# ratt-ru/pfb-clean

Hardware: AMD Instinct MI355X
Metric: PCG matvecs/sec (FFT-conv A^H A apply), 4k x 4k x 8-band cube (higher is better)
Workload: dtype f32; 1 GPU; 4096x4096x8-band cube PCG (hessian_psf + Tikhonov, M = x/sigmainv, tol=0, minit=maxit=20); nx_psf=8192, bands_per_gpu=8, parallelism=band-shard x1, allreduce_hook=False

## Files before the change

### include/pfb_hip.h

```cpp
#ifndef PFB_HIP_H
#define PFB_HIP_H

#include <stddef.h>
#include <stdint.h>

#ifdef __cplusplus
extern "C" {
#endif

#define PFB_ABI_VERSION 1

#define PFB_F32 0
#define PFB_F64 1

#define PFB_OK               0
#define PFB_ERR_INVALID     -1
#define PFB_ERR_UNSUPPORTED -2
#define PFB_ERR_HIP         -3
#define PFB_ERR_NONFINITE   -4
#define PFB_ERR_ALLOC       -5
#define PFB_ERR_COMM        -6

#define PFB_PCG_CONVERGED     0
#define PFB_PCG_MAXIT         1
// ... 60 lines not shown
    double rnorm;
} pfb_pcg_result;

size_t pfb_pcg_work_bytes(const pfb_conv_plan* plan, int nb);
int pfb_pcg_solve(pfb_conv_plan* plan, int band0, int nb,
                  const void* b, void* x, void* r_out,
                  const void* beam, double wsum, double sigmainv, double mdiv,
                  double tol, int maxit, int minit, int backtrack,
                  void* work, pfb_allreduce_fn allreduce, void* allreduce_ctx,
                  pfb_pcg_result* result, void* stream);

size_t pfb_pcg_bands_work_bytes(const pfb_conv_plan* plan, int nb);
int pfb_pcg_solve_bands(pfb_conv_plan* plan, int band0, int nb,
                        const void* b, void* x, void* r_out,
                        const void* beam, double wsum, double sigmainv, double mdiv,
                        double tol, int maxit, int minit, int backtrack,
                        void* work, pfb_pcg_result* results, void* stream);

int pfb_bandmix_dots(int dtype, const void* A, const void* c, int nband, size_t npix, double sigmainv,
                     const void* p, const void* r, void* out, double* dots3, double* ws, void* stream);

size_t pfb_hessparam_work_bytes(const pfb_conv_plan* plan);
int pfb_hessparam_apply(pfb_conv_plan* plan, const void* L, const void* LH, const void* e, double sigmainv,
                        const void* x, void* out, void* work, void* stream);
int pfb_hessparam_apply_dots(pfb_conv_plan* plan, const void* L, const void* LH, const void* e, double sigmainv,
                             const void* x, void* out, const void* dot_with, const void* dot_with2,
                             double* dots_out, void* work, void* stream);

size_t pfb_pcg_param_work_bytes(const pfb_conv_plan* plan, int nb);
int pfb_pcg_solve_param(pfb_conv_plan* plan, int nb, const void* L, const void* LH, const void* e,
                        const void* b, void* x, void* r_out, double sigmainv, double mdiv,
                        double tol, int maxit, int minit, int backtrack,
                        void* work, pfb_pcg_result* result, void* stream);

#define PFB_COMM_ID_BYTES 128
typedef struct pfb_comm pfb_comm;
int pfb_comm_bind(const char* librccl_path);
int pfb_comm_unique_id(void* id128);
int pfb_comm_init(int rank, int nranks, const void* id128, pfb_comm** out);
int pfb_comm_destroy(pfb_comm* comm);
int pfb_comm_info(const pfb_comm* comm, int* rank, int* nranks, int* device, int* rccl_version);
int pfb_comm_allreduce(void* comm, double* dev_buf, int count, void* stream);
int pfb_comm_check(pfb_comm* comm);
int pfb_comm_abort(pfb_comm* comm);

typedef struct pfb_psi_plan pfb_psi_plan;

int pfb_psi_plan_create(int nband, int nx, int ny, int nbasis, const int* basis_k,
                        const double* filters, int nlevel, int dtype,
                        pfb_psi_plan** plan);
int pfb_psi_plan_destroy(pfb_psi_plan* plan);
int pfb_psi_plan_dims(const pfb_psi_plan* plan, int* nymax, int* nxmax);
int pfb_psi_dot(pfb_psi_plan* plan, const void* x, void* alpha, void* stream);
int pfb_psi_hdot(pfb_psi_plan* plan, const void* alpha, void* xo, void* stream);

int pfb_dual_update(int dtype, const void* vp, void* v, const void* weight,
                    double lam, double sigma, int nband, size_t nper,
                    void* vp_out, void* stream);
int pfb_dual_bandsum(int dtype, const void* vp, const void* v, double sigma, int nband,
                     size_t nper, void* sum_out, void* stream);
int pfb_dual_apply(int dtype, const void* vp, void* v, const void* weight, const void* sum_in,
                   double lam, double sigma, int nband, size_t nper, void* vp_out, void* stream);
int pfb_dual_bandsum_chunk(int dtype, const void* vp, const void* v, double sigma, int nband, size_t count,
                           size_t band_stride, void* sum_out, void* stream);
int pfb_dual_apply_chunk(int dtype, const void* vp, void* v, const void* weight, const void* sum_in,
                         double lam, double sigma, int nband, size_t count, size_t band_stride,
// ... 217 lines not shown
```

### pfb_clean_amd/_lib.py

```python
import ctypes as C
import os

_HERE = os.path.dirname(os.path.abspath(__file__))
LIB_PATH = os.environ.get('PFB_HIP_LIB') or os.path.join(_HERE, 'libpfb_hip.so')

PFB_F32, PFB_F64 = 0, 1
PFB_OK = 0
ERRORS = {-1: 'invalid argument', -2: 'unsupported size/dtype', -3: 'HIP runtime error',
          -4: 'non-finite value', -5: 'device allocation failed', -6: 'band-shard exchange failed'}
PCG_STATUS = {0: 'converged', 1: 'maxit', 2: 'zero-residual', 3: 'breakdown'}
REDUCE_WS_DOUBLES = 8192


PFB_ERR_INVALID = -1
PFB_ERR_UNSUPPORTED = -2
PFB_ERR_ALLOC = -5
PFB_ERR_COMM = -6


class PfbHipError(RuntimeError):
    def __init__(self, code, msg):
        super().__init__(f"libpfb_hip: {ERRORS.get(code, code)}: {msg}")
        self.code = code

# ... 13 lines not shown
_vp, _i, _d, _sz = C.c_void_p, C.c_int, C.c_double, C.c_size_t
SIGNATURES = {
    'pfb_abi_version': (_i, []),
    'pfb_last_error': (C.c_char_p, []),
    'pfb_psfconv_plan_create': (_i, [_i, _i, _i, _i, _i, _i, C.POINTER(_vp)]),
    'pfb_psfconv_plan_destroy': (_i, [_vp]),
    'pfb_psfconv_set_psfhat': (_i, [_vp, _vp, _vp]),
    'pfb_psfconv_apply': (_i, [_vp, _i, _i, _vp, _vp, _d, _d, _vp, _vp, _vp, _vp]),
    'pfb_psfconv_set_psf': (_i, [_vp, _vp, _vp, _vp]),
    'pfb_psfhat_regrid': (_i, [_i, _vp, _i, _i, _i, _i, _i, _i, _i, _vp, _vp]),
    'pfb_psfhat_from_psf': (_i, [_i, _vp, _i, _i, _i, _vp, _vp]),
    'pfb_psfconv_apply_dots': (_i, [_vp, _i, _i, _vp, _vp, _d, _d, _vp, _vp, _vp, _vp, _vp]),
    'pfb_psfconv_apply_dots_bands': (_i, [_vp, _i, _i, _vp, _vp, _d, _d, _vp, _vp, _vp, _vp, _vp]),
    'pfb_psfconv_plan_info': (_i, [_vp, C.POINTER(_i), C.POINTER(_i), C.POINTER(_sz)]),
    'pfb_psfconv_set_profiling': (_i, [_vp, _i]),
    'pfb_psfconv_get_profile': (_i, [_vp, C.POINTER(_d), C.POINTER(_i)]),
    'pfb_dot': (_i, [_i, _vp, _vp, _sz, _vp, _vp, _vp]),
    'pfb_norm_diff_sums': (_i, [_i, _vp, _vp, _sz, _vp, _vp, _vp]),
    'pfb_any_nonzero': (_i, [_i, _vp, _sz, _vp, _vp, _vp]),
    'pfb_axpby': (_i, [_i, _d, _vp, _d, _vp, _sz, _vp]),
    'pfb_pcg_work_bytes': (_sz, [_vp, _i]),
    'pfb_pcg_solve': (_i, [_vp, _i, _i, _vp, _vp, _vp, _vp, _d, _d, _d, _d, _i, _i, _i,
                           _vp, ALLREDUCE_FN, _vp, C.POINTER(PcgResult), _vp]),
    'pfb_pcg_bands_work_bytes': (_sz, [_vp, _i]),
    'pfb_pcg_solve_bands': (_i, [_vp, _i, _i, _vp, _vp, _vp, _vp, _d, _d, _d, _d, _i, _i, _i,
                                 _vp, C.POINTER(PcgResult), _vp]),
    'pfb_bandmix_dots': (_i, [_i, _vp, _vp, _i, _sz, _d, _vp, _vp, _vp, _vp, _vp, _vp]),
    'pfb_hessparam_work_bytes': (_sz, [_vp]),
    'pfb_hessparam_apply': (_i, [_vp, _vp, _vp, _vp, _d, _vp, _vp, _vp, _vp]),
    'pfb_hessparam_apply_dots': (_i, [_vp, _vp, _vp, _vp, _d, _vp, _vp, _vp, _vp, _vp, _vp, _vp]),
    'pfb_pcg_param_work_bytes': (_sz, [_vp, _i]),
    'pfb_pcg_solve_param': (_i, [_vp, _i, _vp, _vp, _vp, _vp, _vp, _vp, _d, _d, _d, _i, _i, _i,
                                 _vp, C.POINTER(PcgResult), _vp]),
    'pfb_comm_bind': (_i, [C.c_char_p]),
    'pfb_comm_unique_id': (_i, [_vp]),
    'pfb_comm_init': (_i, [_i, _i, _vp, C.POINTER(_vp)]),
    'pfb_comm_destroy': (_i, [_vp]),
    'pfb_comm_info': (_i, [_vp, C.POINTER(_i), C.POINTER(_i), C.POINTER(_i), C.POINTER(_i)]),
    'pfb_comm_allreduce': (_i, [_vp, _vp, _i, _vp]),
    'pfb_comm_check': (_i, [_vp]),
    'pfb_comm_abort': (_i, [_vp]),
    'pfb_psi_plan_create': (_i, [_i, _i, _i, _i, C.POINTER(_i), C.POINTER(_d), _i, _i,
                                 C.POINTER(_vp)]),
    'pfb_psi_plan_destroy': (_i, [_vp]),
    'pfb_psi_plan_dims': (_i, [_vp, C.POINTER(_i), C.POINTER(_i)]),
    'pfb_psi_dot': (_i, [_vp, _vp, _vp, _vp]),
    'pfb_psi_hdot': (_i, [_vp, _vp, _vp, _vp]),
    'pfb_dual_update': (_i, [_i, _vp, _vp, _vp, _d, _d, _i, _sz, _vp, _vp]),
    'pfb_dual_bandsum': (_i, [_i, _vp, _vp, _d, _i, _sz, _vp, _vp]),
    'pfb_dual_apply': (_i, [_i, _vp, _vp, _vp, _vp, _d, _d, _i, _sz, _vp, _vp]),
    'pfb_prox_21': (_i, [_i, _vp, _vp, _vp, _d, _d, _i, _sz, _vp]),
    'pfb_dual_update_l2': (_i, [_i, _vp, _vp, _vp, _d, _d, _i, _sz, _vp]),
    'pfb_dual_bandsum_chunk': (_i, [_i, _vp, _vp, _d, _i, _sz, _sz, _vp, _vp]),
    'pfb_dual_apply_chunk': (_i, [_i, _vp, _vp, _vp, _vp, _d, _d, _i, _sz, _sz, _vp, _vp]),
    'pfb_clark_subminor': (_i, [_i, _vp, _sz, _i, _vp, _i, _i, _vp, _vp, _vp, _i, _i, _vp, _d, _d, _i, _vp, _vp]),
    'pfb_hogbom': (_i, [_i, _vp, _vp, _vp, _vp, _i, _i, _i, _i, _i, _d, _d, _d, _i, _vp, _sz, _vp, _vp, _vp]),
    'pfb_freqmul': (_i, [_i, _vp, _vp, _vp, _i, _sz, _vp, _vp, _vp]),
    'pfb_prox_21m': (_i, [_i, _vp, _vp, _vp, _d, _d, _i, _sz, _vp]),
    'pfb_pd_primal_update': (_i, [_i, _vp, _vp, _vp, _d, _i, _i, _sz, _vp, _vp, _vp, _vp]),
    'pfb_pd_primal_update2': (_i, [_i, _vp, _vp, _vp, _vp, _vp, _d, _i, _i, _sz, _vp, _vp, _vp, _vp]),
    'pfb_gauss2d': (_i, [_vp, _vp, _sz, _vp, _i, _i, _vp, _vp, _vp, _vp]),
    'pfb_gauss_kernel_grid': (_i, [_i, _vp, _vp, _i, _i, _i, _i, _i, _i, _vp, _vp, _i, _i, _i, _i, _vp, _vp]),
    'pfb_kernel_gather': (_i, [_i, _vp, _i, _i, _i, _i, _i, _i, _i, _i, _i, _vp, _vp]),
    'pfb_kernhat_ratio': (_i, [_vp, _vp, _i, _sz, _vp, _vp]),
    'pfb_comps_work_bytes': (_sz, [_sz]),
    'pfb_comps_mask': (_i, [_i, _vp, _i, _sz, _vp, _vp]),
# ... 88 lines not shown
```

### pfb_clean_amd/csrc/cgvec.hip

```cpp
#include "conv_plan.hpp"
#include "pcg_state.hpp"
#include "entry.hpp"
#include <chrono>
#include <unistd.h>
#include <cstring>
#include <cstdlib>
#include <utility>
#include <vector>

namespace pfb {

constexpr int RED_MAX_GRID = 1024;

static inline int red_grid(size_t nvec) {
    size_t g = (nvec + RED_BLOCK - 1) / RED_BLOCK;
    g = (g + 3) / 4;
    if (g < 1) g = 1;
    if (g > (size_t)RED_MAX_GRID) g = RED_MAX_GRID;
    return (int)g;
}

template <typename T, int V>
__global__ void __launch_bounds__(RED_BLOCK)
k_dot(const T* __restrict__ a, const T* __restrict__ b, size_t nvec, double* __restrict__ ws) {
// ... 122 lines not shown
            acc[2] += (double)xnew * (double)xnew;
        }
        st<T, V>(xn, i, ox);
        st<T, V>(rn, i, orr);
    }
    emit_partials<3>(acc, ws);
}

template <typename T, int V>
__global__ void __launch_bounds__(RED_BLOCK)
k_pcg_dir(T* __restrict__ p, const T* __restrict__ r, const double* __restrict__ beta_dev,
          T mdiv, size_t nvec, double* __restrict__ ws) {
    double acc[1] = {0.0};
    if (beta_dev[S_DEAD - S_BETA] != 0.0) {
        emit_partials<1>(acc, ws);
        return;
    }
    const T beta = (T)beta_dev[0];
    for (size_t i = (size_t)blockIdx.x * blockDim.x + threadIdx.x; i < nvec;
         i += (size_t)gridDim.x * blockDim.x) {
        Pack<T, V> pp = ld<T, V>(p, i), pr = ld<T, V>(r, i);
#pragma unroll
        for (int e = 0; e < V; ++e) {
            const T y = mdiv > T(0) ? pr.e[e] / mdiv : pr.e[e];
            const T v = beta * pp.e[e] - y;
            pp.e[e] = v;
            acc[0] += (v != T(0)) ? 1.0 : 0.0;
        }
        st<T, V>(p, i, pp);
    }
    emit_partials<1>(acc, ws);
}

template <typename T, int V, int U, bool XNT, bool REV>
__global__ void __launch_bounds__(RED_BLOCK)
k_pcg_update_dir(const T* x, const T* r, T* __restrict__ p, const T* __restrict__ Ap, T* xn, T* rn,
                 const double* __restrict__ S, T mdiv, size_t nvs, int gps, double* __restrict__ ws) {
    const int s = blockIdx.x / gps, g = blockIdx.x - s * gps;
    const double* Sb = S + (size_t)s * SB;
    { const size_t off = (size_t)s * nvs * V; x += off; r += off; p += off; Ap += off; xn += off; rn += off; }
    double acc[4] = {0.0, 0.0, 0.0, 0.0};
    if (sys_live(Sb)) {
        const T alpha = (T)Sb[S_ALPHA];
        const T beta = (T)Sb[S_BETA];
        const size_t stride = (size_t)gps * blockDim.x;
        for (size_t i0 = (size_t)g * blockDim.x + threadIdx.x; i0 < nvs; i0 += U * stride) {
            Pack<T, V> px[U], pr[U], pp[U], pa[U];
#pragma unroll
            for (int u = 0; u < U; ++u) {
                const size_t ii = i0 + u * stride;
                const size_t i = REV ? nvs - 1 - ii : ii;
                if (ii < nvs) {
                    px[u] = XNT ? ld_nt<T, V>(x, i) : ld<T, V>(x, i);
                    pr[u] = ld<T, V>(r, i); pp[u] = ld<T, V>(p, i); pa[u] = ld<T, V>(Ap, i);
                }
            }
#pragma unroll
            for (int u = 0; u < U; ++u) {
                const size_t ii = i0 + u * stride;
                const size_t i = REV ? nvs - 1 - ii : ii;
                if (ii >= nvs) break;
                Pack<T, V> ox, orr;
#pragma unroll
                for (int e = 0; e < V; ++e) {
                    const T xnew = px[u].e[e] + alpha * pp[u].e[e];
                    const T rnew = pr[u].e[e] + alpha * pa[u].e[e];
                    const T y = mdiv > T(0) ? rnew / mdiv : rnew;
                    ox.e[e] = xnew;
                    orr.e[e] = rnew;
                    const double d = (double)xnew - (double)px[u].e[e];
                    acc[0] += (double)rnew * (double)y;
                    acc[1] += d * d;
                    acc[2] += (double)xnew * (double)xnew;
                    const T pn = beta * pp[u].e[e] - y;
                    pp[u].e[e] = pn;
                    acc[3] += (pn != T(0)) ? 1.0 : 0.0;
                }
                if constexpr (XNT) st_nt<T, V>(xn, i, ox); else st<T, V>(xn, i, ox);
                st<T, V>(rn, i, orr);
                st<T, V>(p, i, pp[u]);
            }
        }
    } else if (xn != x) {
        for (size_t i = (size_t)g * blockDim.x + threadIdx.x; i < nvs; i += (size_t)gps * blockDim.x) {
            st<T, V>(xn, i, ld<T, V>(x, i));
            st<T, V>(rn, i, ld<T, V>(r, i));
        }
    }
    emit_partials<4>(acc, ws);
}

__global__ void k_set_alpha(double* S) { S[S_ALPHA] = S[S_RHO] / S[S_PAP]; S[S_NBT] = 0.0; }
__global__ void k_scale_alpha(double* S) { S[S_ALPHA] *= 0.75; }
__global__ void k_set_beta(double* S) { S[S_BETA] = S[S_RHON] / S[S_RHO]; }
__global__ void k_accept_rho(double* S) { S[S_RHO] = S[S_RHON]; }

__global__ void __launch_bounds__(256)
k_iter_sums(const double* __restrict__ cp, int bs, int qs, int bst, const double* __restrict__ ws, int gps,
            int have_upd, double* __restrict__ S, double mdiv, int predict, int logic) {
    __shared__ double vals[8];
    const int s = blockIdx.x, w = threadIdx.x >> 6, lane = threadIdx.x & 63;
    if (cp && w < 3) {
        const double* src = cp + (size_t)w * qs + (size_t)s * bst;
        double acc = 0.0;
        for (int k = lane; k < bs; k += 64) acc += src[k];
        acc = wave_sum(acc);
        if (lane == 0) vals[w] = acc;
    }
    if (have_upd && w < 4) {
        const double* src = ws + ((size_t)w * gridDim.x + s) * gps;
        double acc = 0.0;
        for (int g = lane; g < gps; g += 64) acc += src[g];
        acc = wave_sum(acc);
        if (lane == 0) vals[3 + w] = acc;
    }
    __syncthreads();
    double* Sb = S + (size_t)s * SB;
    if (threadIdx.x == 0 && sys_live(Sb)) {
        if (cp) { Sb[S_PAP] = vals[0]; Sb[S_RAP] = vals[1]; Sb[S_APAP] = vals[2]; }
        if (have_upd) { Sb[S_RHON] = vals[3]; Sb[S_NUM] = vals[4]; Sb[S_DEN] = vals[5]; Sb[S_ANY] = vals[6]; }
        if (logic) {
            if (have_upd) iter_end_dev(Sb);
            iter_begin_dev(Sb, mdiv, predict);
        }
    }
}
__global__ void __launch_bounds__(256)
k_iter_end(const double* __restrict__ ws, int gps, double* __restrict__ S) {
    __shared__ double vals[4];
    const int s = blockIdx.x, w = threadIdx.x >> 6, lane = threadIdx.x & 63;
    if (ws) {
        const double* src = ws + ((size_t)w * gridDim.x + s) * gps;
        double acc = 0.0;
        for (int g = lane; g < gps; g += 64) acc += src[g];
        acc = wave_sum(acc);
        if (lane == 0) vals[w] = acc;
        __syncthreads();
    }
    double* Sb = S + (size_t)s * SB;
    if (threadIdx.x == 0 && sys_live(Sb)) {
        if (ws) { Sb[S_RHON] = vals[0]; Sb[S_NUM] = vals[1]; Sb[S_DEN] = vals[2]; Sb[S_ANY] = vals[3]; }
        iter_end_dev(Sb);
    }
}
__global__ void k_iter_begin(double* S, double mdiv, int predict) { iter_begin_dev(S, mdiv, predict); }
__global__ void k_iter_end_begin(double* S, double mdiv, int predict) {
    iter_end_dev(S);
    iter_begin_dev(S, mdiv, predict);
}
__global__ void k_final_check(double* S, int nsys) {
    for (int s = threadIdx.x; s < nsys; s += blockDim.x) {
        double* Sb = S + (size_t)s * SB;
        if (Sb[S_ZERO] == 0.0 && Sb[S_DEAD] == 0.0 && Sb[S_ANY] == 0.0) {
            Sb[S_DEAD] = 1.0; Sb[S_K] -= 1.0; Sb[S_EPS] = Sb[S_EPSP];
        }
    }
}

#define PFB_LAUNCH_VEC(T, kern, n, ptrs, ...)                                              \
    do {                                                                                   \
        if (can_vec<T>(n, ptrs)) {                                                         \
            const size_t nvec = (n) / V16<T>::N;                                           \
            const int G = red_grid(nvec);                                                  \
            G_used = G;                                                                    \
            hipLaunchKernelGGL((kern<T, V16<T>::N>), dim3(G), dim3(RED_BLOCK), 0, st,      \
                               __VA_ARGS__, nvec, ws);                                     \
        } else {                                                                           \
            const int G = red_grid(n);                                                     \
            G_used = G;                                                                    \
            hipLaunchKernelGGL((kern<T, 1>), dim3(G), dim3(RED_BLOCK), 0, st, __VA_ARGS__, \
                               (size_t)(n), ws);                                           \
        }                                                                                  \
    } while (0)

template <typename T>
static int dot_impl(const void* a, const void* b, size_t n, double* out, double* ws, hipStream_t st) {
    int G_used = 0;
    using PL = std::initializer_list<const void*>;
    PFB_LAUNCH_VEC(T, k_dot, n, (PL{a, b}), (const T*)a, (const T*)b);
    return final_sum(ws, G_used, 1, out, st);
}
// ... 19 lines not shown
        hipLaunchKernelGGL((k_axpby<T, V16<T>::N>), dim3(red_grid(nvec)), dim3(RED_BLOCK), 0, st,
                           (T)a, (const T*)x, (T)b, (T*)y, nvec);
    } else {
        hipLaunchKernelGGL((k_axpby<T, 1>), dim3(red_grid(n)), dim3(RED_BLOCK), 0, st,
                           (T)a, (const T*)x, (T)b, (T*)y, n);
    }
    PFB_HIP_CHECK(hipGetLastError());
    return PFB_OK;
}

static int stream_grid(size_t nvec) {
    const int ncu = device_cu_count();
    size_t g = (nvec + RED_BLOCK - 1) / RED_BLOCK;
    g = (g + 3) / 4;
    if (g < 1) g = 1;
    if (g > (size_t)ncu) g = ncu;
    return (int)g;
}
static int update_grid(size_t nvs, int nsys) {
    int g = stream_grid(nvs);
    const int share = stream_grid((size_t)1 << 40) / nsys;
    if (g > share) g = share;
    if (g > RED_MAX_GRID / nsys) g = RED_MAX_GRID / nsys;
    return g < 1 ? 1 : g;
}
static int init_grid(size_t nvs, int nsys) {
    int g = red_grid(nvs);
    if (g > RED_MAX_GRID / nsys) g = RED_MAX_GRID / nsys;
    return g < 1 ? 1 : g;
}

struct PcgLayout {
    static constexpr size_t NONE = ~(size_t)0;
    size_t r, p, Ap, S, ws, xalt = NONE, ralt = NONE, tmp = NONE, mixp = NONE, total = 0;
    PcgLayout(const pfb_conv_plan* plan, int nb, int nsys, bool alternates, bool param) {
        auto take = [&](size_t bytes) { const size_t at = total; total += bytes; return at; };
        const size_t vb = vec_bytes(plan, nb);
        r = take(vb); p = take(vb); Ap = take(vb);
        S = take(((size_t)nsys * SB * sizeof(double) + 255) & ~(size_t)255);
        ws = take(sizeof(double) * 4 * (size_t)(nsys > RED_MAX_GRID ? nsys : RED_MAX_GRID));
        if (alternates) { xalt = take(vb); ralt = take(vb); }
        if (param) { const MixWork mw(plan); tmp = take(mw.total); mixp = tmp + mw.partials; }
    }
    template <typename U> U* at(void* work, size_t off) const { return off == NONE ? nullptr : (U*)((char*)work + off); }
};

struct PcgSync {
    pfb_allreduce_fn allreduce;
    void* actx;
    hipStream_t st;
    hipEvent_t ev = nullptr;
    double comm_timeout = 600.0;
    ~PcgSync() { if (ev) (void)hipEventDestroy(ev); }
    int open() {
        if (!allreduce) return PFB_OK;
        set_error("%s", "");
        if (const char* e = getenv("PFB_COMM_TIMEOUT_S")) { const double v = atof(e); if (v > 0) comm_timeout = v; }
        PFB_HIP_CHECK(hipEventCreateWithFlags(&ev, hipEventDisableTiming));
        return PFB_OK;
    }
    int comm_fail(const char* what) {
        char msg[384];
        snprintf(msg, sizeof(msg), "%s", pfb_last_error());
        (void)allreduce(actx, nullptr, -1, (void*)st);
        set_error("pcg: %s%s%s -- exchange aborted, this rank's result is void", what, msg[0] ? ": " : "", msg);
        return PFB_ERR_COMM;
    }
    int reduce(double* buf, int count) {
        if (allreduce && allreduce(actx, buf, count, (void*)st) != 0) return comm_fail("the all-reduce hook failed");
        return PFB_OK;
    }
    int wait_event(hipEvent_t e) {
        if (!allreduce) { PFB_HIP_CHECK(hipEventSynchronize(e)); return PFB_OK; }
        const auto t0 = std::chrono::steady_clock::now();
        for (long spins = 0;; ++spins) {
            const hipError_t q = hipEventQuery(e);
            if (q == hipSuccess) return PFB_OK;
            if (q != hipErrorNotReady) { set_error("pcg: hipEventQuery -> %s", hipGetErrorString(q)); return PFB_ERR_HIP; }
            if (spins < 4096) continue;
            if (allreduce(actx, nullptr, 0, (void*)st) != 0) return comm_fail("the exchange reported a failure");
            const double el = std::chrono::duration<double>(std::chrono::steady_clock::now() - t0).count();
            if (el > comm_timeout) {
                char what[128];
                snprintf(what, sizeof(what), "no progress on the solver's stream for %.0f s (PFB_COMM_TIMEOUT_S)", el);
                set_error("%s", "");
                return comm_fail(what);
            }
            usleep(el < 0.01 ? 20 : 500);
        }
    }
    int wait_stream() {
        if (!allreduce) { PFB_HIP_CHECK(hipStreamSynchronize(st)); return PFB_OK; }
        PFB_HIP_CHECK(hipEventRecord(ev, st));
        return wait_event(ev);
    }
    int fetch(double* h, const double* S, size_t count) {
        PFB_HIP_CHECK(hipMemcpyAsync(h, S, sizeof(double) * count, hipMemcpyDeviceToHost, st));
        return wait_stream();
    }
};

struct PcgSolve {
    pfb_conv_plan* plan;
    int band0, nb;
    bool per_band;
    const void* b; void* x; void* r_out; const void* beam;
    double wsum, sigmainv, mdiv, tol;
    int maxit, minit, backtrack;
    size_t lookahead_max;
    void* work;
    pfb_allreduce_fn allreduce; void* actx;
    const void *L, *LH;
    pfb_pcg_result* res;
    hipStream_t st;
};

template <typename T>
struct PcgOp {
    pfb_conv_plan* plan;
    int band0, nb, bps;
    size_t ns;
    bool per_band;
    const T* beam;
    double wsum, sigmainv;
    const T *Lm, *LHm;
    T* tmp;
    double* mixp;
    hipStream_t st;
    struct Partials { const double* cp; int bs, qs, bst; };

    int mix(const T* v, T* out, const T* rr, double* partials, int* G) const {
        return hessparam_apply_partials(plan, Lm, LHm, beam, sigmainv, v, out, rr, tmp, partials, G, st);
    }
    int apply(const T* x0, T* r) const {
// ... 6 lines not shown
            const int err = mix(p, Ap, rc, mixp, &G);
            *w = {mixp, G, G, 0};
            return err;
        }
        const size_t off = (size_t)lo * ns;
        w->cp = plan->partials;
        return psfconv_apply_partials(plan, band0 + lo * bps, nl * bps, p + off, beam ? beam + off : nullptr, wsum,
                                      sigmainv, Ap + off, p + off, rc + off, per_band, &w->bs, &w->qs, &w->bst, (void*)st);
    }
    int apply_dot(const T* p, T* Ap, double* pap) const {
        if (!Lm) return pfb_psfconv_apply(plan, band0, nb, p, beam, wsum, sigmainv, Ap, p, pap, (void*)st);
        int G = 0;
        const int err = mix(p, Ap, nullptr, mixp, &G);
        if (err == PFB_OK)
            hipLaunchKernelGGL(k_final_sum<RED_BLOCK>, dim3(1), dim3(RED_BLOCK), 0, st, (const double*)mixp, G, 1, pap);
        return err;
    }
};

template <typename T>
struct Pcg {
    pfb_conv_plan* plan;
    int nb;
    const T* b; T* x; T* r_out;
    double mdiv_d, tol;
    int maxit, minit;
    PcgSync sync;
    hipStream_t st;
    int nsys;
    size_t n, ns, nvs;
    bool vec;
    T *r, *p, *Ap, *xalt, *ralt;
    double *S, *ws;
    T mdiv;
    std::vector<double> h;
    PcgOp<T> A;

    explicit Pcg(const PcgSolve& q)
        : plan(q.plan), nb(q.nb), b((const T*)q.b), x((T*)q.x), r_out((T*)q.r_out), mdiv_d(q.mdiv), tol(q.tol),
          maxit(q.maxit), minit(q.minit), sync{q.allreduce, q.actx, q.st}, st(q.st), nsys(q.per_band ? q.nb : 1),
          mdiv((T)q.mdiv), h((size_t)nsys * SB) {
        n = (size_t)nb * plan->nx * plan->ny;
        ns = n / nsys;
        const PcgLayout lay(plan, nb, nsys, !q.per_band, q.L != nullptr);
        r = lay.at<T>(q.work, lay.r); p = lay.at<T>(q.work, lay.p); Ap = lay.at<T>(q.work, lay.Ap);
        S = lay.at<double>(q.work, lay.S); ws = lay.at<double>(q.work, lay.ws);
        xalt = lay.at<T>(q.work, lay.xalt); ralt = lay.at<T>(q.work, lay.ralt);
        A = {plan, q.band0, nb, nb / nsys, ns, q.per_band, (const T*)q.beam, q.wsum, q.sigmainv, (const T*)q.L,
             (const T*)q.LH, lay.at<T>(q.work, lay.tmp), lay.at<double>(q.work, lay.mixp), st};
        using PL = std::initializer_list<const void*>;
        vec = can_vec<T>(ns, PL{x, b, r, p, Ap});
        nvs = vec ? ns / V16<T>::N : ns;
    }

    int init() {
        int err;
        if ((err = sync.open()) != PFB_OK) return err;
        PFB_HIP_CHECK(hipMemsetAsync(S, 0, sizeof(double) * h.size(), st));
        if ((err = A.apply(x, r)) != PFB_OK) return err;
        const int gps = init_grid(nvs, nsys);
        if (vec)
            hipLaunchKernelGGL((k_pcg_init<T, V16<T>::N>), dim3(nsys * gps), dim3(RED_BLOCK), 0, st, r, b, p, mdiv, nvs,
                               gps, ws);
        else
            hipLaunchKernelGGL((k_pcg_init<T, 1>), dim3(nsys * gps), dim3(RED_BLOCK), 0, st, r, b, p, mdiv, nvs, gps, ws);
        const int hook = sync.allreduce ? 1 : 0;
        hipLaunchKernelGGL(k_init_state, dim3(nsys), dim3(RED_BLOCK), 0, st, (const double*)ws, gps, S, tol,
                           (double)minit, (double)maxit, 1, 1 - hook);
        if (hook) {
            if ((err = sync.reduce(S + S_RHON, 2)) != PFB_OK) return err;
            hipLaunchKernelGGL(k_init_state, dim3(nsys), dim3(RED_BLOCK), 0, st, (const double*)ws, gps, S, tol,
                               (double)minit, (double)maxit, 0, 1);
        }
        PFB_HIP_CHECK(hipGetLastError());
        return sync.fetch(h.data(), S, h.size());
    }

    int run(int predict, size_t lookahead_max) {
        const size_t nS = h.size();
        const bool hook = sync.allreduce != nullptr;
        auto any_live = [&](const double* hs) {
            for (int s = 0; s < nsys; ++s) if (sys_live(hs + (size_t)s * SB)) return true;
            return false;
        };
        int err;
        bool lookahead = n <= lookahead_max;
        if (const char* la = getenv("PFB_PCG_LOOKAHEAD")) lookahead = atoi(la) != 0;
        if (lookahead && plan->pcg_pin_n < nsys) {
            if (plan->pcg_pin) { PFB_HIP_CHECK(hipStreamSynchronize(st)); (void)hipHostFree(plan->pcg_pin); }
            plan->pcg_pin = nullptr;
            plan->pcg_pin_n = 0;
            PFB_HIP_CHECK(hipHostMalloc((void**)&plan->pcg_pin, sizeof(double) * 2 * nS, hipHostMallocDefault));
            plan->pcg_pin_n = nsys;
            for (int e = 0; e < 2; ++e)
                if (!plan->pcg_ev[e]) PFB_HIP_CHECK(hipEventCreateWithFlags(&plan->pcg_ev[e], hipEventDisableTiming));
        }
        const bool xnt = vec && n * sizeof(T) >= ((size_t)32 << 20);
        const double* seen = h.data();
        bool go = (1.0 > tol || 0 < minit) && 0 < maxit && any_live(seen);
        int khost = 0, slot = 0;
        bool pending_end = false, have_prev = false;
        int lo = 0, nl = nsys, gpl = update_grid(nvs, nsys);
        T *xc = x, *rc = r, *xn = xalt ? xalt : x, *rn = ralt ? ralt : r;
        auto narrow = [&](const double* hs) {
            int a = 0, z = nsys;
            while (a < z && !sys_live(hs + (size_t)a * SB)) ++a;
            while (z > a && !sys_live(hs + (size_t)(z - 1) * SB)) --z;
            if (z > a && (a != lo || z - a != nl)) { lo = a; nl = z - a; gpl = update_grid(nvs, nl); }
        };
        while (go) {
            const size_t off = (size_t)lo * ns;
            double* Sl = S + (size_t)lo * SB;
            typename PcgOp<T>::Partials c;
            if ((err = A.apply_partials(p, Ap, rc, lo, nl, &c)) != PFB_OK) return err;
            hipLaunchKernelGGL(k_iter_sums, dim3(nl), dim3(256), 0, st, c.cp, c.bs, c.qs, c.bst,
                               (const double*)ws, gpl, pending_end ? 1 : 0, Sl, mdiv_d, predict, hook ? 0 : 1);
            if (hook) {
                if ((err = sync.reduce(Sl + S_PAP, pending_end ? 7 : 4)) != PFB_OK) return err;
                if (pending_end) hipLaunchKernelGGL(k_iter_end_begin, dim3(1), dim3(1), 0, st, Sl, mdiv_d, predict);
                else hipLaunchKernelGGL(k_iter_begin, dim3(1), dim3(1), 0, st, Sl, mdiv_d, predict);
            }
            pending_end = false;
#define PFB_UPDATE(VV, XN)                                                                                     \
            hipLaunchKernelGGL((k_pcg_update_dir<T, VV, 2, XN, XN>), dim3(nl * gpl), dim3(RED_BLOCK), 0, st,   \
                               (const T*)xc + off, (const T*)rc + off, p + off, (const T*)Ap + off, xn + off,    \
                               rn + off, (const double*)Sl, mdiv, nvs, gpl, ws)
            if (xnt) PFB_UPDATE(V16<T>::N, true);
            else if (vec) PFB_UPDATE(V16<T>::N, false);
            else PFB_UPDATE(1, false);
#undef PFB_UPDATE
            std::swap(xc, xn);
            std::swap(rc, rn);
            if (khost + 1 < minit && khost + 1 < maxit) {
                pending_end = true;
            } else {
                if (hook) {
                    hipLaunchKernelGGL(k_iter_sums, dim3(nl), dim3(256), 0, st, (const double*)nullptr, 0, 0, 0,
                                       (const double*)ws, gpl, 1, Sl, mdiv_d, predict, 0);
                    if ((err = sync.reduce(Sl + S_RHON, 3)) != PFB_OK) return err;
                }
                hipLaunchKernelGGL(k_iter_end, dim3(nl), dim3(256), 0, st, hook ? nullptr : (const double*)ws, gpl, Sl);
            }
            PFB_HIP_CHECK(hipGetLastError());
            ++khost;
            if (khost < minit && khost < maxit) continue;
            if (lookahead && khost < maxit) {
                double* snap = plan->pcg_pin + (size_t)slot * nS;
                PFB_HIP_CHECK(hipMemcpyAsync(snap, S, sizeof(double) * nS, hipMemcpyDeviceToHost, st));
                PFB_HIP_CHECK(hipEventRecord(plan->pcg_ev[slot], st));
                if (have_prev) {
                    if ((err = sync.wait_event(plan->pcg_ev[slot ^ 1])) != PFB_OK) return err;
                    seen = plan->pcg_pin + (size_t)(slot ^ 1) * nS;
                    go = any_live(seen);
                    if (go) narrow(seen);
                }
                have_prev = true;
                slot ^= 1;
                continue;
            }
            if ((err = sync.fetch(h.data(), S, nS)) != PFB_OK) return err;
            seen = h.data();
            go = khost < maxit && any_live(seen);
            if (go) narrow(seen);
        }
        bool check = false;
        for (int s = 0; s < nsys; ++s) check |= seen[(size_t)s * SB + S_DEAD] == 0.0 && seen[(size_t)s * SB + S_ZERO] == 0.0;
        if (check) {
            if ((err = sync.reduce(S + S_ANY, 1)) != PFB_OK) return err;
            hipLaunchKernelGGL(k_final_check, dim3(1), dim3(64), 0, st, S, nsys);
            PFB_HIP_CHECK(hipGetLastError());
        }
        if (xc != x) PFB_HIP_CHECK(hipMemcpyAsync(x, xc, n * sizeof(T), hipMemcpyDeviceToDevice, st));
        if (r_out) PFB_HIP_CHECK(hipMemcpyAsync(r_out, rc, n * sizeof(T), hipMemcpyDeviceToDevice, st));
        return sync.fetch(h.data(), S, nS);
    }

    int run_exact() {
        using PL = std::initializer_list<const void*>;
        T *xcur = x, *rcur = r, *xnew = xalt, *rnew = ralt;
        int err, G_used = 0, k = 0, nbt = 0;
        double eps = 1.0, rho = h[S_RHO];
        bool broke = false;
        while (h[S_ZERO] == 0.0 && (eps > tol || k < minit) && k < maxit) {
            if ((err = A.apply_dot(p, Ap, S + S_PAP)) != PFB_OK) return err;
            if ((err = sync.reduce(S + S_PAP, 1)) != PFB_OK) return err;
            hipLaunchKernelGGL(k_set_alpha, dim3(1), dim3(1), 0, st, S);
            for (;;) {
                PFB_LAUNCH_VEC(T, k_pcg_update, n, (PL{xcur, rcur, p, Ap, xnew, rnew}), (const T*)xcur,
                               (const T*)rcur, (const T*)p, (const T*)Ap, xnew, rnew,
                               (const double*)(S + S_ALPHA), mdiv);
                hipLaunchKernelGGL(k_final_sum<RED_BLOCK>, dim3(1), dim3(RED_BLOCK), 0, st, ws, G_used, 3, S + S_RHON);
                if ((err = sync.reduce(S + S_RHON, 3)) != PFB_OK) return err;
                if ((err = sync.fetch(h.data(), S, S_NSCALAR)) != PFB_OK) return err;
                if (!(h[S_RHON] > rho)) break;
                hipLaunchKernelGGL(k_scale_alpha, dim3(1), dim3(1), 0, st, S);
                ++nbt;
            }
            { T* t = xcur; xcur = xnew; xnew = t; t = rcur; rcur = rnew; rnew = t; }
            hipLaunchKernelGGL(k_set_beta, dim3(1), dim3(1), 0, st, S);
            PFB_LAUNCH_VEC(T, k_pcg_dir, n, (PL{p, rcur}), p, (const T*)rcur, (const double*)(S + S_BETA), mdiv);
            hipLaunchKernelGGL(k_final_sum<RED_BLOCK>, dim3(1), dim3(RED_BLOCK), 0, st, ws, G_used, 1, S + S_ANY);
            if ((err = sync.reduce(S + S_ANY, 1)) != PFB_OK) return err;
            hipLaunchKernelGGL(k_accept_rho, dim3(1), dim3(1), 0, st, S);
            rho = h[S_RHON];
            const double num = h[S_NUM], den = h[S_DEN];
            if ((err = sync.fetch(h.data(), S, S_NSCALAR)) != PFB_OK) return err;
            if (h[S_ANY] == 0.0) { broke = true; break; }
// ... 5 lines not shown
        if (r_out) PFB_HIP_CHECK(hipMemcpyAsync(r_out, rcur, n * sizeof(T), hipMemcpyDeviceToDevice, st));
        if ((err = sync.wait_stream()) != PFB_OK) return err;
        PFB_HIP_CHECK(hipGetLastError());
        return PFB_OK;
    }

    void report(pfb_pcg_result* res) const {
        for (int s = 0; s < nsys; ++s) {
            const double* Sb = h.data() + (size_t)s * SB;
            pfb_pcg_result& o = res[s];
            o.rnorm = Sb[S_RHO];
            if (Sb[S_ZERO] != 0.0) {
                o.status = PFB_PCG_ZERO_RESIDUAL;
                o.matvecs = 1;
                o.eps = 1.0;
                continue;
            }
            const int k = (int)Sb[S_K];
            const bool dead = Sb[S_DEAD] != 0.0;
            o.status = dead ? PFB_PCG_BREAKDOWN : (k >= maxit ? PFB_PCG_MAXIT : PFB_PCG_CONVERGED);
            o.iters = k;
            o.eps = Sb[S_EPS];
            o.backtracks = (int)Sb[S_NBTSUM];
            o.matvecs = 1 + k + (dead ? 1 : 0);
        }
    }
};

template <typename T>
static int pcg_solve(const PcgSolve& q) {
    Pcg<T> s(q);
    PFB_REQUIRE(!q.allreduce || s.nsys == 1, PFB_ERR_INVALID, "pcg: an all-reduce hook needs the bands to be one system");
    memset(q.res, 0, sizeof(*q.res) * s.nsys);
    int err = s.init();
    if (err == PFB_OK) err = q.backtrack == 1 ? s.run_exact() : s.run(q.backtrack == 2 ? 2 : 3, q.lookahead_max);
    if (err == PFB_OK) s.report(q.res);
    return err;
}

static int pcg_checked(const char* who, const PcgSolve& q) {
    PFB_REQUIRE(q.plan && q.b && q.x && q.work && q.res, PFB_ERR_INVALID, "%s: null argument", who);
    PFB_REQUIRE(q.band0 >= 0 && q.nb > 0 && q.band0 + q.nb <= q.plan->nband, PFB_ERR_INVALID,
                "%s: band range [%d,%d) outside plan", who, q.band0, q.band0 + q.nb);
    PFB_REQUIRE((reinterpret_cast<uintptr_t>(q.work) & 255u) == 0, PFB_ERR_INVALID,
                "%s: work must be 256-byte aligned", who);
    return q.plan->dtype == PFB_F32 ? pcg_solve<float>(q) : pcg_solve<double>(q);
}

}

using namespace pfb;

extern "C" {

int pfb_dot(int dtype, const void* a, const void* b, size_t n, double* out, double* ws, void* stream) {
    PFB_REQUIRE(a && b && out && ws, PFB_ERR_INVALID, "dot: null argument");
    return dtype == PFB_F32 ? dot_impl<float>(a, b, n, out, ws, as_stream(stream))
                            : dot_impl<double>(a, b, n, out, ws, as_stream(stream));
}

int pfb_norm_diff_sums(int dtype, const void* x, const void* xp, size_t n, double* out, double* ws,
                       void* stream) {
    PFB_REQUIRE(x && xp && out && ws, PFB_ERR_INVALID, "norm_diff_sums: null argument");
    return dtype == PFB_F32 ? nd_impl<float>(x, xp, n, out, ws, as_stream(stream))
                            : nd_impl<double>(x, xp, n, out, ws, as_stream(stream));
}
// ... 11 lines not shown
}
size_t pfb_pcg_work_bytes(const pfb_conv_plan* plan, int nb) {
    if (!plan || nb <= 0) return 0;
    return PcgLayout(plan, nb, 1, true, false).total;
}

int pfb_pcg_solve(pfb_conv_plan* plan, int band0, int nb, const void* b, void* x, void* r_out,
                  const void* beam, double wsum, double sigmainv, double mdiv, double tol,
                  int maxit, int minit, int backtrack, void* work, pfb_allreduce_fn allreduce,
                  void* allreduce_ctx, pfb_pcg_result* result, void* stream) {
    return pcg_checked("pcg_solve", {plan, band0, nb, false, b, x, r_out, beam, wsum, sigmainv, mdiv, tol, maxit, minit,
                                     backtrack, (size_t)4 << 20, work, allreduce, allreduce_ctx, nullptr, nullptr, result,
                                     as_stream(stream)});
}

size_t pfb_pcg_param_work_bytes(const pfb_conv_plan* plan, int nb) {
    if (!plan || nb != plan->nband) return 0;
    return PcgLayout(plan, nb, 1, true, true).total;
}

int pfb_pcg_solve_param(pfb_conv_plan* plan, int nb, const void* L, const void* LH, const void* e, const void* b,
                        void* x, void* r_out, double sigmainv, double mdiv, double tol, int maxit, int minit,
                        int backtrack, void* work, pfb_pcg_result* result, void* stream) {
    PFB_REQUIRE(plan && L && LH, PFB_ERR_INVALID, "pcg_solve_param: null argument");
    PFB_REQUIRE(nb == plan->nband, PFB_ERR_INVALID,
                "pcg_solve_param: the band mix couples all %d bands of the plan, nb = %d", plan->nband, nb);
    PFB_REQUIRE(nb <= 16, PFB_ERR_UNSUPPORTED, "pcg_solve_param: nband %d > 16", nb);
    PFB_REQUIRE(backtrack >= 0 && backtrack <= 2, PFB_ERR_INVALID, "pcg_solve_param: backtrack must be 0, 1 or 2");
    return pcg_checked("pcg_solve_param", {plan, 0, nb, false, b, x, r_out, e, 0.5, sigmainv, mdiv, tol, maxit, minit,
                                           backtrack, (size_t)4 << 20, work, nullptr, nullptr, L, LH, result,
                                           as_stream(stream)});
}

size_t pfb_pcg_bands_work_bytes(const pfb_conv_plan* plan, int nb) {
    if (!plan || nb <= 0) return 0;
    return PcgLayout(plan, nb, nb, false, false).total;
}

int pfb_pcg_solve_bands(pfb_conv_plan* plan, int band0, int nb, const void* b, void* x, void* r_out,
                        const void* beam, double wsum, double sigmainv, double mdiv, double tol,
                        int maxit, int minit, int backtrack, void* work, pfb_pcg_result* results, void* stream) {
    PFB_REQUIRE(backtrack != 1, PFB_ERR_UNSUPPORTED,
                "pcg_solve_bands: backtrack=1 (the exact loop) is not batched; solve band by band with pfb_pcg_solve");
    PFB_REQUIRE(backtrack == 0 || backtrack == 2, PFB_ERR_INVALID, "pcg_solve_bands: backtrack must be 0 or 2");
    return pcg_checked("pcg_solve_bands", {plan, band0, nb, true, b, x, r_out, beam, wsum, sigmainv, mdiv, tol, maxit,
                                           minit, backtrack, (size_t)16 << 20, work, nullptr, nullptr, nullptr, nullptr,
                                           results, as_stream(stream)});
}

}
```

Measured before the change: 438.4 cube-matvecs/s.

## Fuse per-iteration scalar reductions into update kernel and update x/r in place

New measurement: 433.3 cube-matvecs/s. 0.988x the previous value.

```diff
diff --git a/include/pfb_hip.h b/include/pfb_hip.h
--- a/include/pfb_hip.h
+++ b/include/pfb_hip.h
@@ -116,6 +116,8 @@
                         const void* b, void* x, void* r_out, double sigmainv, double mdiv,
                         double tol, int maxit, int minit, int backtrack,
                         void* work, pfb_pcg_result* result, void* stream);
+
+void pfb_pcg_debug_counts(int* counts6);
 
 #define PFB_COMM_ID_BYTES 128
 typedef struct pfb_comm pfb_comm;
diff --git a/pfb_clean_amd/_lib.py b/pfb_clean_amd/_lib.py
--- a/pfb_clean_amd/_lib.py
+++ b/pfb_clean_amd/_lib.py
@@ -69,6 +69,7 @@
     'pfb_pcg_param_work_bytes': (_sz, [_vp, _i]),
     'pfb_pcg_solve_param': (_i, [_vp, _i, _vp, _vp, _vp, _vp, _vp, _vp, _d, _d, _d, _i, _i, _i,
                                  _vp, C.POINTER(PcgResult), _vp]),
+    'pfb_pcg_debug_counts': (None, [C.POINTER(_i)]),
     'pfb_comm_bind': (_i, [C.c_char_p]),
     'pfb_comm_unique_id': (_i, [_vp]),
     'pfb_comm_init': (_i, [_i, _i, _vp, C.POINTER(_vp)]),
diff --git a/pfb_clean_amd/csrc/cgvec.hip b/pfb_clean_amd/csrc/cgvec.hip
--- a/pfb_clean_amd/csrc/cgvec.hip
+++ b/pfb_clean_amd/csrc/cgvec.hip
@@ -178,12 +178,53 @@
     emit_partials<1>(acc, ws);
 }
 
+struct IterScalars {
+    const double* cp; int bs, qs, bst;
+    const double* ws; int gps;
+    int sum_upd, end, begin;
+    double mdiv; int predict;
+};
+__device__ __forceinline__ void iter_scalars_dev(const IterScalars& q, int s, int nl, double* Sb, double* vals) {
+    const int w = threadIdx.x >> 6, lane = threadIdx.x & 63;
+    if (q.cp && w < 3) {
+        const double* src = q.cp + (size_t)w * q.qs + (size_t)s * q.bst;
+        double acc = 0.0;
+        for (int k = lane; k < q.bs; k += 64) acc += src[k];
+        acc = wave_sum(acc);
+        if (lane == 0) vals[w] = acc;
+    }
+    if (q.sum_upd && w < 4) {
+        const double* src = q.ws + ((size_t)w * nl + s) * q.gps;
+        double acc = 0.0;
+        for (int g = lane; g < q.gps; g += 64) acc += src[g];
+        acc = wave_sum(acc);
+        if (lane == 0) vals[3 + w] = acc;
+    }
+    __syncthreads();
+    if (threadIdx.x == 0 && sys_live(Sb)) {
+        if (q.cp) { Sb[S_PAP] = vals[0]; Sb[S_RAP] = vals[1]; Sb[S_APAP] = vals[2]; }
+        if (q.sum_upd) { Sb[S_RHON] = vals[3]; Sb[S_NUM] = vals[4]; Sb[S_DEN] = vals[5]; Sb[S_ANY] = vals[6]; }
+        if (q.end) iter_end_dev(Sb);
+        if (q.begin) iter_begin_dev(Sb, q.mdiv, q.predict);
+    }
+}
+__global__ void __launch_bounds__(256)
+k_iter_sums(IterScalars q, double* __restrict__ S) {
+    __shared__ double vals[8];
+    iter_scalars_dev(q, blockIdx.x, gridDim.x, S + (size_t)blockIdx.x * SB, vals);
+}
+
 template <typename T, int V, int U, bool XNT, bool REV>
 __global__ void __launch_bounds__(RED_BLOCK)
 k_pcg_update_dir(const T* x, const T* r, T* __restrict__ p, const T* __restrict__ Ap, T* xn, T* rn,
-                 const double* __restrict__ S, T mdiv, size_t nvs, int gps, double* __restrict__ ws) {
+                 const double* __restrict__ Sin, double* __restrict__ Sout, IterScalars q, T mdiv, size_t nvs, int gps,
+                 double* __restrict__ ws) {
+    __shared__ double Sb[SB], vals[8];
     const int s = blockIdx.x / gps, g = blockIdx.x - s * gps;
-    const double* Sb = S + (size_t)s * SB;
+    if (threadIdx.x < SB) Sb[threadIdx.x] = Sin[(size_t)s * SB + threadIdx.x];
+    iter_scalars_dev(q, s, gridDim.x / gps, Sb, vals);
+    __syncthreads();
+    if (g == 0 && threadIdx.x < SB) Sout[(size_t)s * SB + threadIdx.x] = Sb[threadIdx.x];
     { const size_t off = (size_t)s * nvs * V; x += off; r += off; p += off; Ap += off; xn += off; rn += off; }
     double acc[4] = {0.0, 0.0, 0.0, 0.0};
     if (sys_live(Sb)) {
@@ -242,36 +283,6 @@
 __global__ void k_accept_rho(double* S) { S[S_RHO] = S[S_RHON]; }
 
 __global__ void __launch_bounds__(256)
-k_iter_sums(const double* __restrict__ cp, int bs, int qs, int bst, const double* __restrict__ ws, int gps,
-            int have_upd, double* __restrict__ S, double mdiv, int predict, int logic) {
-    __shared__ double vals[8];
-    const int s = blockIdx.x, w = threadIdx.x >> 6, lane = threadIdx.x & 63;
-    if (cp && w < 3) {
-        const double* src = cp + (size_t)w * qs + (size_t)s * bst;
-        double acc = 0.0;
-        for (int k = lane; k < bs; k += 64) acc += src[k];
-        acc = wave_sum(acc);
-        if (lane == 0) vals[w] = acc;
-    }
-    if (have_upd && w < 4) {
-        const double* src = ws + ((size_t)w * gridDim.x + s) * gps;
-        double acc = 0.0;
-        for (int g = lane; g < gps; g += 64) acc += src[g];
-        acc = wave_sum(acc);
-        if (lane == 0) vals[3 + w] = acc;
-    }
-    __syncthreads();
-    double* Sb = S + (size_t)s * SB;
-    if (threadIdx.x == 0 && sys_live(Sb)) {
-        if (cp) { Sb[S_PAP] = vals[0]; Sb[S_RAP] = vals[1]; Sb[S_APAP] = vals[2]; }
-        if (have_upd) { Sb[S_RHON] = vals[3]; Sb[S_NUM] = vals[4]; Sb[S_DEN] = vals[5]; Sb[S_ANY] = vals[6]; }
-        if (logic) {
-            if (have_upd) iter_end_dev(Sb);
-            iter_begin_dev(Sb, mdiv, predict);
-        }
-    }
-}
-__global__ void __launch_bounds__(256)
 k_iter_end(const double* __restrict__ ws, int gps, double* __restrict__ S) {
     __shared__ double vals[4];
     const int s = blockIdx.x, w = threadIdx.x >> 6, lane = threadIdx.x & 63;
@@ -288,11 +299,6 @@
         if (ws) { Sb[S_RHON] = vals[0]; Sb[S_NUM] = vals[1]; Sb[S_DEN] = vals[2]; Sb[S_ANY] = vals[3]; }
         iter_end_dev(Sb);
     }
-}
-__global__ void k_iter_begin(double* S, double mdiv, int predict) { iter_begin_dev(S, mdiv, predict); }
-__global__ void k_iter_end_begin(double* S, double mdiv, int predict) {
-    iter_end_dev(S);
-    iter_begin_dev(S, mdiv, predict);
 }
 __global__ void k_final_check(double* S, int nsys) {
     for (int s = threadIdx.x; s < nsys; s += blockDim.x) {
@@ -378,13 +384,14 @@
 
 struct PcgLayout {
     static constexpr size_t NONE = ~(size_t)0;
-    size_t r, p, Ap, S, ws, xalt = NONE, ralt = NONE, tmp = NONE, mixp = NONE, total = 0;
+    size_t r, p, Ap, S, ws, ws_doubles, xalt = NONE, ralt = NONE, tmp = NONE, mixp = NONE, total = 0;
     PcgLayout(const pfb_conv_plan* plan, int nb, int nsys, bool alternates, bool param) {
         auto take = [&](size_t bytes) { const size_t at = total; total += bytes; return at; };
         const size_t vb = vec_bytes(plan, nb);
         r = take(vb); p = take(vb); Ap = take(vb);
-        S = take(((size_t)nsys * SB * sizeof(double) + 255) & ~(size_t)255);
-        ws = take(sizeof(double) * 4 * (size_t)(nsys > RED_MAX_GRID ? nsys : RED_MAX_GRID));
+        S = take((2 * (size_t)nsys * SB * sizeof(double) + 255) & ~(size_t)255);
+        ws_doubles = 4 * (size_t)(nsys > RED_MAX_GRID ? nsys : RED_MAX_GRID);
+        ws = take(2 * sizeof(double) * ws_doubles);
         if (alternates) { xalt = take(vb); ralt = take(vb); }
         if (param) { const MixWork mw(plan); tmp = take(mw.total); mixp = tmp + mw.partials; }
     }
@@ -446,6 +453,15 @@
     }
 };
 
+constexpr size_t INPLACE_MIN_BYTES = (size_t)64 << 20;
+static size_t inplace_min_bytes() {
+    const char* e = getenv("PFB_PCG_INPLACE_MIN_BYTES");
+    return e && *e ? (size_t)strtoull(e, nullptr, 10) : INPLACE_MIN_BYTES;
+}
+
+struct PcgCounts { int applies, updates, scalars, copies, gps, bs; };
+static thread_local PcgCounts pcg_counts;
+
 struct PcgSolve {
     pfb_conv_plan* plan;
     int band0, nb;
@@ -518,6 +534,10 @@
     bool vec;
     T *r, *p, *Ap, *xalt, *ralt;
     double *S, *ws;
+    size_t ws_doubles;
+    int cur = 0;
+    double* Sc(int c) const { return S + (size_t)c * h.size(); }
+    double* wsc(int c) const { return ws + (size_t)c * ws_doubles; }
     T mdiv;
     std::vector<double> h;
     PcgOp<T> A;
@@ -530,7 +550,7 @@
         ns = n / nsys;
         const PcgLayout lay(plan, nb, nsys, !q.per_band, q.L != nullptr);
         r = lay.at<T>(q.work, lay.r); p = lay.at<T>(q.work, lay.p); Ap = lay.at<T>(q.work, lay.Ap);
-        S = lay.at<double>(q.work, lay.S); ws = lay.at<double>(q.work, lay.ws);
+        S = lay.at<double>(q.work, lay.S); ws = lay.at<double>(q.work, lay.ws); ws_doubles = lay.ws_doubles;
         xalt = lay.at<T>(q.work, lay.xalt); ralt = lay.at<T>(q.work, lay.ralt);
         A = {plan, q.band0, nb, nb / nsys, ns, q.per_band, (const T*)q.beam, q.wsum, q.sigmainv, (const T*)q.L,
              (const T*)q.LH, lay.at<T>(q.work, lay.tmp), lay.at<double>(q.work, lay.mixp), st};
@@ -542,7 +562,7 @@
     int init() {
         int err;
         if ((err = sync.open()) != PFB_OK) return err;
-        PFB_HIP_CHECK(hipMemsetAsync(S, 0, sizeof(double) * h.size(), st));
+        PFB_HIP_CHECK(hipMemsetAsync(S, 0, sizeof(double) * 2 * h.size(), st));
         if ((err = A.apply(x, r)) != PFB_OK) return err;
         const int gps = init_grid(nvs, nsys);
         if (vec)
@@ -587,78 +607,99 @@
         int khost = 0, slot = 0;
         bool pending_end = false, have_prev = false;
         int lo = 0, nl = nsys, gpl = update_grid(nvs, nsys);
-        T *xc = x, *rc = r, *xn = xalt ? xalt : x, *rn = ralt ? ralt : r;
+        const bool inplace = !xalt || n * sizeof(T) >= inplace_min_bytes();
+        T *xc = x, *rc = r, *xn = inplace ? x : xalt, *rn = inplace ? r : ralt;
         auto narrow = [&](const double* hs) {
             int a = 0, z = nsys;
             while (a < z && !sys_live(hs + (size_t)a * SB)) ++a;
             while (z > a && !sys_live(hs + (size_t)(z - 1) * SB)) --z;
-            if (z > a && (a != lo || z - a != nl)) { lo = a; nl = z - a; gpl = update_grid(nvs, nl); }
+            if (!(z > a && (a != lo || z - a != nl))) return hipSuccess;
+            lo = a; nl = z - a; gpl = update_grid(nvs, nl);
+            return hipMemcpyAsync(Sc(cur ^ 1), Sc(cur), sizeof(double) * nS, hipMemcpyDeviceToDevice, st);
         };
         while (go) {
             const size_t off = (size_t)lo * ns;
-            double* Sl = S + (size_t)lo * SB;
+            double *Sl = Sc(cur) + (size_t)lo * SB, *Sn = Sc(cur ^ 1) + (size_t)lo * SB;
             typename PcgOp<T>::Partials c;
             if ((err = A.apply_partials(p, Ap, rc, lo, nl, &c)) != PFB_OK) return err;
-            hipLaunchKernelGGL(k_iter_sums, dim3(nl), dim3(256), 0, st, c.cp, c.bs, c.qs, c.bst,
-                               (const double*)ws, gpl, pending_end ? 1 : 0, Sl, mdiv_d, predict, hook ? 0 : 1);
+            ++pcg_counts.applies;
+            pcg_counts.gps = gpl;
+            pcg_counts.bs = c.bs;
+            IterScalars q{c.cp, c.bs, c.qs, c.bst, wsc(cur), gpl, pending_end ? 1 : 0, pending_end ? 1 : 0, 1, mdiv_d,
+                          predict};
             if (hook) {
+                IterScalars qsum = q;
+                qsum.end = qsum.begin = 0;
+                hipLaunchKernelGGL(k_iter_sums, dim3(nl), dim3(256), 0, st, qsum, Sl);
+                ++pcg_counts.scalars;
                 if ((err = sync.reduce(Sl + S_PAP, pending_end ? 7 : 4)) != PFB_OK) return err;
-                if (pending_end) hipLaunchKernelGGL(k_iter_end_begin, dim3(1), dim3(1), 0, st, Sl, mdiv_d, predict);
-                else hipLaunchKernelGGL(k_iter_begin, dim3(1), dim3(1), 0, st, Sl, mdiv_d, predict);
+                q.cp = nullptr;
+                q.sum_upd = 0;
             }
             pending_end = false;
 #define PFB_UPDATE(VV, XN)                                                                                     \
             hipLaunchKernelGGL((k_pcg_update_dir<T, VV, 2, XN, XN>), dim3(nl * gpl), dim3(RED_BLOCK), 0, st,   \
                                (const T*)xc + off, (const T*)rc + off, p + off, (const T*)Ap + off, xn + off,    \
-                               rn + off, (const double*)Sl, mdiv, nvs, gpl, ws)
+                               rn + off, (const double*)Sl, Sn, q, mdiv, nvs, gpl, wsc(cur ^ 1))
             if (xnt) PFB_UPDATE(V16<T>::N, true);
             else if (vec) PFB_UPDATE(V16<T>::N, false);
             else PFB_UPDATE(1, false);
 #undef PFB_UPDATE
+            ++pcg_counts.updates;
+            cur ^= 1;
             std::swap(xc, xn);
             std::swap(rc, rn);
             if (khost + 1 < minit && khost + 1 < maxit) {
                 pending_end = true;
             } else {
                 if (hook) {
-                    hipLaunchKernelGGL(k_iter_sums, dim3(nl), dim3(256), 0, st, (const double*)nullptr, 0, 0, 0,
-                                       (const double*)ws, gpl, 1, Sl, mdiv_d, predict, 0);
-                    if ((err = sync.reduce(Sl + S_RHON, 3)) != PFB_OK) return err;
+                    hipLaunchKernelGGL(k_iter_sums, dim3(nl), dim3(256), 0, st,
+                                       IterScalars{nullptr, 0, 0, 0, wsc(cur), gpl, 1, 0, 0, mdiv_d, predict}, Sn);
+                    if ((err = sync.reduce(Sn + S_RHON, 3)) != PFB_OK) return err;
+                    ++pcg_counts.scalars;
                 }
-                hipLaunchKernelGGL(k_iter_end, dim3(nl), dim3(256), 0, st, hook ? nullptr : (const double*)ws, gpl, Sl);
+                hipLaunchKernelGGL(k_iter_end, dim3(nl), dim3(256), 0, st, hook ? nullptr : (const double*)wsc(cur), gpl,
+                                   Sn);
+                ++pcg_counts.scalars;
             }
             PFB_HIP_CHECK(hipGetLastError());
             ++khost;
             if (khost < minit && khost < maxit) continue;
             if (lookahead && khost < maxit) {
                 double* snap = plan->pcg_pin + (size_t)slot * nS;
-                PFB_HIP_CHECK(hipMemcpyAsync(snap, S, sizeof(double) * nS, hipMemcpyDeviceToHost, st));
+                PFB_HIP_CHECK(hipMemcpyAsync(snap, Sc(cur), sizeof(double) * nS, hipMemcpyDeviceToHost, st));
                 PFB_HIP_CHECK(hipEventRecord(plan->pcg_ev[slot], st));
                 if (have_prev) {
                     if ((err = sync.wait_event(plan->pcg_ev[slot ^ 1])) != PFB_OK) return err;
                     seen = plan->pcg_pin + (size_t)(slot ^ 1) * nS;
                     go = any_live(seen);
-                    if (go) narrow(seen);
+                    if (go) PFB_HIP_CHECK(narrow(seen));
                 }
                 have_prev = true;
                 slot ^= 1;
                 continue;
             }
-            if ((err = sync.fetch(h.data(), S, nS)) != PFB_OK) return err;
+            if ((err = sync.fetch(h.data(), Sc(cur), nS)) != PFB_OK) return err;
             seen = h.data();
             go = khost < maxit && any_live(seen);
-            if (go) narrow(seen);
+            if (go) PFB_HIP_CHECK(narrow(seen));
         }
         bool check = false;
         for (int s = 0; s < nsys; ++s) check |= seen[(size_t)s * SB + S_DEAD] == 0.0 && seen[(size_t)s * SB + S_ZERO] == 0.0;
         if (check) {
-            if ((err = sync.reduce(S + S_ANY, 1)) != PFB_OK) return err;
-            hipLaunchKernelGGL(k_final_check, dim3(1), dim3(64), 0, st, S, nsys);
+            if ((err = sync.reduce(Sc(cur) + S_ANY, 1)) != PFB_OK) return err;
+            hipLaunchKernelGGL(k_final_check, dim3(1), dim3(64), 0, st, Sc(cur), nsys);
             PFB_HIP_CHECK(hipGetLastError());
         }
-        if (xc != x) PFB_HIP_CHECK(hipMemcpyAsync(x, xc, n * sizeof(T), hipMemcpyDeviceToDevice, st));
-        if (r_out) PFB_HIP_CHECK(hipMemcpyAsync(r_out, rc, n * sizeof(T), hipMemcpyDeviceToDevice, st));
-        return sync.fetch(h.data(), S, nS);
+        if (xc != x) {
+            PFB_HIP_CHECK(hipMemcpyAsync(x, xc, n * sizeof(T), hipMemcpyDeviceToDevice, st));
+            ++pcg_counts.copies;
+        }
+        if (r_out) {
+            PFB_HIP_CHECK(hipMemcpyAsync(r_out, rc, n * sizeof(T), hipMemcpyDeviceToDevice, st));
+            ++pcg_counts.copies;
+        }
+        return sync.fetch(h.data(), Sc(cur), nS);
     }
 
     int run_exact() {
@@ -730,6 +771,7 @@
     Pcg<T> s(q);
     PFB_REQUIRE(!q.allreduce || s.nsys == 1, PFB_ERR_INVALID, "pcg: an all-reduce hook needs the bands to be one system");
     memset(q.res, 0, sizeof(*q.res) * s.nsys);
+    pcg_counts = {};
     int err = s.init();
     if (err == PFB_OK) err = q.backtrack == 1 ? s.run_exact() : s.run(q.backtrack == 2 ? 2 : 3, q.lookahead_max);
     if (err == PFB_OK) s.report(q.res);
@@ -807,6 +849,13 @@
                                            as_stream(stream)});
 }
 
+void pfb_pcg_debug_counts(int* counts6) {
+    if (!counts6) return;
+    counts6[0] = pcg_counts.applies; counts6[1] = pcg_counts.updates;
+    counts6[2] = pcg_counts.scalars; counts6[3] = pcg_counts.copies;
+    counts6[4] = pcg_counts.gps; counts6[5] = pcg_counts.bs;
+}
+
 size_t pfb_pcg_bands_work_bytes(const pfb_conv_plan* plan, int nb) {
     if (!plan || nb <= 0) return 0;
     return PcgLayout(plan, nb, nb, false, false).total;
```
